# jiahuei/sparse-image-captioning

Hardware: AMD Instinct MI355X
Metric: captions/sec (higher is better)
Workload: dtype bf16; 1 GPU; configs[1]: ORT dense, 256 images x 5 captions, teacher-forcing XE fwd+bwd+clip+Adam; images_per_gpu=256, regions=36, captions_per_image=5, parallelism=single

## Files before the change

include/ortk.h:

```cpp
#ifndef ORTK_H
#define ORTK_H

#include <stddef.h>
#include <stdint.h>

#ifdef __cplusplus
extern "C" {
#endif

#define ORTK_VERSION 14
#define ORTK_EINVAL (-1)
#define ORTK_ENOSPC (-2)
#define ORTK_ENOSYS (-3)
#define ORTK_EEXCHANGE (-4)

typedef void* ortk_stream;

int ortk_version(void);
int ortk_device_ok(void);

struct ortk_sparse_plan;
typedef struct ortk_config {
    int32_t d_model, d_ff, n_layers, n_heads;
    int32_t vocab, feat, seq_len;
    int32_t pad_id, bos_id, eos_id, unk_id;
    int32_t box_trig;
    int32_t precision;
    float   drop_src, drop;
    int32_t share_enc[16], share_dec[16];
    int32_t share_att_enc, share_att_dec;
    int32_t no_box;
    const struct ortk_sparse_plan* sparse_fwd;
    const struct ortk_sparse_plan* sparse_bwd;
} ortk_config;

int64_t ortk_arena_numel(const ortk_config* cfg);
int64_t ortk_arena_numel_with_buffers(const ortk_config* cfg);
int32_t ortk_arena_entries(const ortk_config* cfg);
int ortk_arena_entry(const ortk_config* cfg, int32_t index, char* name_buf, int64_t* offset,
                     int64_t* numel, int32_t* ndim, int64_t* shape, int32_t* kind);

uint32_t ortk_dropout_site_seed(uint64_t seed, int32_t stack, int32_t layer, int32_t k);

// ... 97 lines not shown
typedef struct ortk_bchain_args {
    const void* w16t; const ortk_chain_unit* units_dev; int32_t n_units;
    void* packed; size_t packed_bytes;
    int64_t M;
    int32_t nin; const void* ain; int64_t ld_ain; const void* dz0;
    const float *xa, *sta, *ga, *dresa; float *dxa, *daa, *dba; void* dza; uint32_t seed_a; int32_t mask_a;
    int32_t NC; const void* hgate; void* gh; float gate_scale;
    const float *xb, *stb, *gb, *dresb; float *dxb, *dab, *dbb; void* dzb; uint32_t seed_b; int32_t mask_b;
    int32_t n2; void* out2;
    float drop_p, eps;
    const int32_t* drop_rows;
} ortk_bchain_args;
int ortk_row_bchain(const ortk_bchain_args* a, ortk_stream stream);

typedef struct ortk_tuning {
    int32_t gemm_t64;
    int32_t attn_impl;
    int32_t attn16_min_lq;
    int32_t side_stream;
    int32_t row_chain;
    int32_t chain_wide;
    int32_t spmm_alias;
    int32_t f32_split;
    int32_t wgrad_wgs;
    int32_t wgrad_group;
    int32_t wgrad_group_splitk;
    int32_t wgrad_group_wgs;
    int32_t wgrad_group_tail;
    int32_t feats_bf16;
    int32_t ln_fuse;
    int32_t samp_epilogue;
    int32_t gemm_epilogue;
    int32_t attn16_short;
} ortk_tuning;
void ortk_get_tuning(ortk_tuning* out);
int ortk_set_tuning(const ortk_tuning* t);

#define ORTK_DEC_UNFUSED 1
#define ORTK_DEC_STACK 2
#define ORTK_DEC_SPARSE_STREAM 4
#define ORTK_DEC_STACK_RB20 8
#define ORTK_DEC_STACK_SPLIT 16
#define ORTK_DEC_SPLIT_SMALL 32
#define ORTK_DEC_SPARSE_GATHER 64
#define ORTK_DEC_STACK_FP8 128
#define ORTK_MAX_BEAM 32
typedef struct ortk_decode_opts {
    int32_t beam_size;
    int32_t num_random_sample;
    float   temperature;
    int32_t decoding_constraint;
    int32_t length_penalty;
    double  length_alpha;
    uint64_t seed;
    const struct ortk_sparse_plan* sparse;
    int32_t exec_flags;
    int32_t with_greedy;
    int64_t sample_row_offset;
    int32_t train;
    uint64_t drop_seed;
    const void* memory;
    int32_t top_k;
    float   top_p;
    int32_t group_size;
    float   diversity_lambda;
} ortk_decode_opts;
// ... 195 lines not shown
```

sparse-image-captioning_amd/_lib.py:

```python
import ctypes as C
import os

import torch

_HERE = os.path.dirname(os.path.abspath(__file__))
LIB_PATH = os.path.join(_HERE, "libortk.so")


class OrtkUnavailable(RuntimeError):
    pass


class OrtkError(RuntimeError):
    pass


class Config(C.Structure):
    _fields_ = [("d_model", C.c_int32), ("d_ff", C.c_int32), ("n_layers", C.c_int32), ("n_heads", C.c_int32),
                ("vocab", C.c_int32), ("feat", C.c_int32), ("seq_len", C.c_int32),
                ("pad_id", C.c_int32), ("bos_id", C.c_int32), ("eos_id", C.c_int32), ("unk_id", C.c_int32),
                ("box_trig", C.c_int32), ("precision", C.c_int32), ("drop_src", C.c_float), ("drop", C.c_float),
                ("share_enc", C.c_int32 * 16), ("share_dec", C.c_int32 * 16),
                ("share_att_enc", C.c_int32), ("share_att_dec", C.c_int32), ("no_box", C.c_int32),
                ("sparse_fwd", C.c_void_p), ("sparse_bwd", C.c_void_p)]
# ... 50 lines not shown
                ("M", C.c_int64),
                ("nin", C.c_int32), ("ain", C.c_void_p), ("ld_ain", C.c_int64), ("dz0", C.c_void_p),
                ("xa", C.c_void_p), ("sta", C.c_void_p), ("ga", C.c_void_p), ("dresa", C.c_void_p), ("dxa", C.c_void_p), ("daa", C.c_void_p),
                ("dba", C.c_void_p), ("dza", C.c_void_p), ("seed_a", C.c_uint32), ("mask_a", C.c_int32),
                ("NC", C.c_int32), ("hgate", C.c_void_p), ("gh", C.c_void_p), ("gate_scale", C.c_float),
                ("xb", C.c_void_p), ("stb", C.c_void_p), ("gb", C.c_void_p), ("dresb", C.c_void_p), ("dxb", C.c_void_p), ("dab", C.c_void_p),
                ("dbb", C.c_void_p), ("dzb", C.c_void_p), ("seed_b", C.c_uint32), ("mask_b", C.c_int32),
                ("n2", C.c_int32), ("out2", C.c_void_p), ("drop_p", C.c_float), ("eps", C.c_float), ("drop_rows", C.c_void_p)]


class MaskedAdamArgs(C.Structure):
    _fields_ = [("w", C.c_void_p), ("g", C.c_void_p), ("mw", C.c_void_p), ("vw", C.c_void_p),
                ("ml", C.c_void_p), ("mm", C.c_void_p), ("mv", C.c_void_p),
                ("draws", C.c_void_p), ("active", C.c_void_p), ("extra_coef", C.c_void_p),
                ("n", C.c_int64), ("index0", C.c_int64), ("mode", C.c_int32), ("seed", C.c_uint32),
                ("lr_w", C.c_float), ("eps_w", C.c_float), ("lr_m", C.c_float), ("eps_m", C.c_float),
                ("beta1", C.c_float), ("beta2", C.c_float), ("clip", C.c_float), ("bc1", C.c_float), ("bc2", C.c_float)]


OPT_ADAM, OPT_SGD, OPT_SGDM, OPT_SGDMOM, OPT_RMSPROP, OPT_ADAGRAD = range(6)
OPT_KINDS = {"adam": OPT_ADAM, "sgd": OPT_SGD, "sgdm": OPT_SGDM, "sgdmom": OPT_SGDMOM, "rmsprop": OPT_RMSPROP, "adagrad": OPT_ADAGRAD}


class OptimArgs(C.Structure):
    _fields_ = [("p", C.c_void_p), ("g", C.c_void_p), ("s1", C.c_void_p), ("s2", C.c_void_p), ("n", C.c_int64),
                ("kind", C.c_int32), ("first_step", C.c_int32), ("zero_grad", C.c_int32),
                ("lr", C.c_float), ("weight_decay", C.c_float), ("alpha", C.c_float), ("beta", C.c_float), ("eps", C.c_float),
                ("clip", C.c_float), ("bc1", C.c_float), ("bc2", C.c_float)]


class Tuning(C.Structure):
    _fields_ = [("gemm_t64", C.c_int32), ("attn_impl", C.c_int32), ("attn16_min_lq", C.c_int32),
                ("side_stream", C.c_int32), ("row_chain", C.c_int32), ("chain_wide", C.c_int32), ("spmm_alias", C.c_int32), ("f32_split", C.c_int32), ("wgrad_wgs", C.c_int32),
                ("wgrad_group", C.c_int32), ("wgrad_group_splitk", C.c_int32), ("wgrad_group_wgs", C.c_int32), ("wgrad_group_tail", C.c_int32), ("feats_bf16", C.c_int32), ("ln_fuse", C.c_int32), ("samp_epilogue", C.c_int32), ("gemm_epilogue", C.c_int32), ("attn16_short", C.c_int32)]


MAX_BEAM = 32
DEC_UNFUSED, DEC_STACK, DEC_SPARSE_STREAM, DEC_STACK_RB20, DEC_STACK_SPLIT, DEC_SPLIT_SMALL, DEC_SPARSE_GATHER, DEC_STACK_FP8 = 1, 2, 4, 8, 16, 32, 64, 128


class DecodeOpts(C.Structure):
    _fields_ = [("beam_size", C.c_int32), ("num_random_sample", C.c_int32), ("temperature", C.c_float),
                ("decoding_constraint", C.c_int32), ("length_penalty", C.c_int32), ("length_alpha", C.c_double),
                ("seed", C.c_uint64), ("sparse", C.POINTER(EllPlanStruct)), ("exec_flags", C.c_int32), ("with_greedy", C.c_int32), ("sample_row_offset", C.c_int64),
                ("train", C.c_int32), ("drop_seed", C.c_uint64), ("memory", C.c_void_p), ("top_k", C.c_int32), ("top_p", C.c_float),
                ("group_size", C.c_int32), ("diversity_lambda", C.c_float)]


class GemmArgs(C.Structure):
    _fields_ = [("A", C.c_void_p), ("B", C.c_void_p), ("C", C.c_void_p),
                ("lda", C.c_int64), ("ldb", C.c_int64), ("ldc", C.c_int64),
                ("M", C.c_int32), ("N", C.c_int32), ("K", C.c_int32), ("transA", C.c_int32), ("transB", C.c_int32),
                ("bias", C.c_void_p), ("rowscale", C.c_void_p), ("resid", C.c_void_p), ("ldr", C.c_int64),
                ("gate", C.c_void_p), ("ldg", C.c_int64), ("gate_scale", C.c_float),
                ("relu", C.c_int32), ("drop_p", C.c_float), ("drop_seed", C.c_uint32),
                ("accumulate", C.c_int32), ("splitk", C.c_int32), ("precision", C.c_int32),
                ("a_dtype", C.c_int32), ("b_dtype", C.c_int32), ("c_dtype", C.c_int32), ("gate_dtype", C.c_int32),
                ("colsum", C.c_void_p), ("drop_row_stride", C.c_int32), ("drop_row_off", C.c_int32),
                ("ln_mode", C.c_int32), ("ln_y_dtype", C.c_int32),
                ("ln_a", C.c_void_p), ("ln_b", C.c_void_p), ("ln_y", C.c_void_p), ("ln_stats", C.c_void_p), ("ln_eps", C.c_float),
                ("ln_x", C.c_void_p), ("ln_dres", C.c_void_p), ("ln_da", C.c_void_p), ("ln_db", C.c_void_p),
                ("tile_stats", C.c_void_p), ("stat_ncols", C.c_int32), ("drop_rows", C.c_void_p),
                ("tile_samp", C.c_void_p), ("samp_seq", C.c_void_p), ("samp_seed", C.c_uint64), ("samp_row_offset", C.c_int64),
                ("samp_L", C.c_int32), ("samp_t", C.c_int32), ("samp_greedy_stride", C.c_int32), ("samp_sample", C.c_int32),
                ("samp_fast", C.c_int32), ("samp_no_store", C.c_int32), ("samp_inv_temperature", C.c_float)]


# ... 90 lines not shown
    "ortk_colsum": (_I32, [_P, _I32, _I64, _P, _I64, _I32, _P]),
    "ortk_gate_apply": (_I32, [_P, _P, _P, _I32, _I64, _F, _P]),
    "ortk_dropout_apply": (_I32, [_P, _P, _I32, _I64, _F, _U32, _P]),
    "ortk_dropout_apply_rows": (_I32, [_P, _P, _I32, _I64, _I32, _F, _U32, _P, _P]),
    "ortk_dropout_site_seed": (_U32, [_U64, _I32, _I32, _I32]),
    "ortk_cast_bf16": (_I32, [_P, _P, _I64, _P]),
    "ortk_fp8_rows": (_I32, [_P, _I64, _I64, _I64, _P, _I64, _P, _P, _I64, _P]),
    "ortk_fill": (_I32, [_P, _I64, _F, _P]),
    "ortk_sum_scratch_floats": (_I64, [_I64]),
    "ortk_sum": (_I32, [_P, _I64, _P, _P, _P]),
    "ortk_adam_clip": (_I32, [_P, _P, _P, _P, _I64, _F, _F, _F, _F, _F, _F, _F, _P]),
    "ortk_adam_clip_zero": (_I32, [_P, _P, _P, _P, _I64, _F, _F, _F, _F, _F, _F, _F, _P]),
    "ortk_optim_states": (_I32, [_I32]),
    "ortk_optim_step": (_I32, [C.POINTER(OptimArgs), _P]),
    "ortk_mask_apply": (_I32, [_P, _P, _P, _I64, _I32, _U32, _P]),
    "ortk_mask_bwd": (_I32, [_P, _P, _P, _P, _P, _I64, _I32, _U32, _P, _P]),
    "ortk_masked_adam_step": (_I32, [C.POINTER(MaskedAdamArgs), _P]),
    "ortk_mask_count": (_I32, [_P, _I64, _I32, _P, _P]),
    "ortk_mask_select_workspace_bytes": (_SZ, [_I32, _I32, _I32, _I32]),
    "ortk_mask_select": (_I32, [_P, _P, _P, _P, _P, _P, _P, _P, _P, _I32, _I32, _I32, _I32, _P, _SZ, _P]),
    "ortk_mask_apply_draws": (_I32, [_P, _P, _P, _P, _I64, _P]),
    "ortk_mask_bwd_draws": (_I32, [_P, _P, _P, _P, _P, _P, _I64, _P, _P]),
    "ortk_decode_step_workspace_bytes": (_SZ, [_CFG, _I32]),
    "ortk_project_memory": (_I32, [_CFG, _P, _P, _I64, _P, _SZ, _P, _P]),
    "ortk_decode_step": (_I32, [_CFG, _P, _P, _I32, _I32, _I32, _I32, _P, _P, _P, _P, _I32, _P, _SZ, _P, _I64, _P]),
    "ortk_axpy_cols": (_I32, [_P, _P, _I32, _I64, _I64, _I32, _P]),
    "ortk_linear_block": (_I32, [_CFG, _I32, C.POINTER(C.c_int64), C.POINTER(C.c_int32), C.POINTER(C.c_int32)]),
    "ortk_sparse_build": (_I32, [C.POINTER(EllPlanStruct), _P, _I32, _P]),
    "ortk_spmm": (_I32, [C.POINTER(EllPlanStruct), _I32, C.POINTER(SpmmArgs), _P]),
    "ortk_spmm_plan": (_I32, [C.POINTER(EllPlanStruct), _I32, C.POINTER(SpmmArgs), C.c_char_p, _I32]),
}

_lib = None
ABI_VERSION = 14


def lib():
    global _lib
    if _lib is None:
        if not os.path.exists(LIB_PATH):
            raise OrtkUnavailable(
                f"{LIB_PATH} is missing: build it with `python -c 'import __graft_entry__ as g; g.build()'` "
                "(or `make -C sparse-image-captioning_amd/csrc`).  There is no CPU / PyTorch fallback.")
        h = C.CDLL(LIB_PATH)
        h.ortk_version.restype = C.c_int32
        if h.ortk_version() != ABI_VERSION:
            raise OrtkUnavailable(
                f"{LIB_PATH} is ABI version {h.ortk_version()}, these bindings were written for version {ABI_VERSION} (include/ortk.h: "
                "ORTK_VERSION): a stale build.  Rebuild it with `make -C sparse-image-captioning_amd/csrc`.")
        for name, (res, args) in SIGNATURES.items():
            fn = getattr(h, name)
            fn.restype = res
            fn.argtypes = args
        _lib = h
    return _lib


def set_tuning(**kw):
    t = Tuning()
    lib().ortk_get_tuning(C.byref(t))
    old = {f: getattr(t, f) for f, _ in Tuning._fields_}
    for k, v in kw.items():
        assert k in old, k
        setattr(t, k, int(v))
    check(lib().ortk_set_tuning(C.byref(t)), "ortk_set_tuning")
    return old

# ... 50 lines not shown
```

sparse-image-captioning_amd/csrc/ortk_attn16.hip:

```cpp
#include <cstdlib>
#include "ortk_internal.h"

namespace {

constexpr int P16 = 72;

__device__ __forceinline__ void wsync() { __builtin_amdgcn_fence(__ATOMIC_ACQ_REL, "wavefront"); __builtin_amdgcn_wave_barrier(); }

template <int NJT> struct KeyGeo {
    static constexpr int KJ = NJT <= 2 ? 32 : NJT <= 4 ? 64 : NJT <= 6 ? 96 : 128;
    static constexpr int PJ = NJT <= 4 ? P16 : 136;
};

template <int PITCH = P16>
__device__ __forceinline__ bf16x8 frag_row(const __bf16* img, int row, int k0) {
    return *reinterpret_cast<const bf16x8*>(img + row * PITCH + k0);
}
template <int PITCH = P16>
__device__ __forceinline__ bf16x8 frag_tr(const __bf16* img, int k0, int x0, int lane) {
    const int lr = lane & 15, lq = lane >> 4;
    const __bf16* p = img + (k0 + 8 * lq + (lr >> 2)) * PITCH + x0 + 4 * (lane & 3);
    typedef bf16x4 __attribute__((address_space(3))) * lds4;
    const bf16x4 lo = __builtin_amdgcn_ds_read_tr16_b64_v4bf16((lds4)(p));
    const bf16x4 hi = __builtin_amdgcn_ds_read_tr16_b64_v4bf16((lds4)(p + 4 * PITCH));
// ... 237 lines not shown
        const int i = it * 16 + lr;
        iv[it] = i < Lqg;
        prow[it] = (((int64_t)g * a.H + h) * Lq + i) * Lk;
        drow[it] = prow[it];
        if (a.drop_p > 0.f && a.drop_rows && a.q_off && iv[it])
            drow[it] = (((int64_t)g * a.H + h) * Lq + ((int64_t)a.drop_rows[qrow0 + i] - (int64_t)g * Lq)) * Lk;
#pragma unroll
        for (int ks = 0; ks < NKS; ++ks) qf[it][ks] = (bf16x8){0, 0, 0, 0, 0, 0, 0, 0};
        if (iv[it]) {
            const __bf16* qp = aq + (qrow0 + i) * a.ldq + h * DK + 8 * lq;
#pragma unroll
            for (int ks = 0; ks < NKS; ++ks) qf[it][ks] = ld_frag(qp + 32 * ks);
        }
        ld_keys4<NJT>(bias4[it], a.bias, a.bias && iv[it], prow[it], Lk, lq);
    }
    stage32_st<DKT>(sV, vreg, lane);
    if (lane < 32) sMask[lane] = mk;
    for (int idx = lane; idx < 16 * (KJS / 4); idx += 64)
        *reinterpret_cast<bf16x4*>(sP + (idx / (KJS / 4)) * PJS + (idx % (KJS / 4)) * 4) = cvt4(make_float4(0.f, 0.f, 0.f, 0.f));
    wsync();
    const float inv_keep = a.drop_p > 0.f ? 1.f / (1.f - a.drop_p) : 1.f;
#pragma unroll
    for (int it = 0; it < 2; ++it) {
        if (it * 16 >= Lqg) break;
        fwd16_tile<NJT, DKT, PJS>(a, kf, qf[it], bias4[it], sMask, sV, sP, lane, it * 16 + lr, iv[it], prow[it], drow[it],
                                  qrow0 + it * 16 + lr, h, inv_keep);
        wsync();
    }
}
static int key_kj(int njt) { return njt <= 2 ? 32 : njt <= 4 ? 64 : njt <= 6 ? 96 : 128; }
static int key_pj(int njt) { return njt <= 4 ? P16 : 136; }
static size_t fwd16_lds(int njt, int nw, int dk) {
    return ((size_t)(16 * njt + key_kj(njt)) * (dk + 8) + (size_t)16 * nw * key_pj(njt)) * sizeof(__bf16) + 128 * sizeof(float);
}

template <int NJT, int DKT, int PJ, typename VF>
__device__ __forceinline__ void bwd16_tile1(const ortk_attn_args& a, const VF& vfr, const bf16x8 (&gf)[DKT / 32], const float4 (&praw)[NJT],
                                            const __bf16* sK, __bf16* sS, __bf16* sD, int lane, int i, bool iv,
                                            int64_t prow, int64_t drow, int64_t qrow, int h, float inv_keep) {
    constexpr int DK = DKT, PD = DKT + 8, KJ = KeyGeo<NJT>::KJ;
    const float qscale = DKT == 64 ? 0.125f : 0.17677669529663687f;
    const int lq = lane >> 4, Lk = a.Lk;
    const bool vec_p = (Lk & 3) == 0;
    f32x4 dp[NJT], pp[NJT];
    float dot = 0.f;
#pragma unroll
    for (int jt = 0; jt < NJT; ++jt) {
        dp[jt] = (f32x4){0.f, 0.f, 0.f, 0.f};
#pragma unroll
        for (int ks = 0; ks < DK / 32; ++ks) dp[jt] = mma(vfr(jt, ks), gf[ks], dp[jt]);
        const int j0 = 16 * jt + 4 * lq;
        const float pv[4] = {praw[jt].x, praw[jt].y, praw[jt].z, praw[jt].w};
        float pd[4];
        bool kp[4] = {true, true, true, true};
        if (a.drop_p > 0.f) ortk_keep4(a.drop_seed, (uint64_t)(drow + j0), a.drop_p, kp);
#pragma unroll
        for (int r = 0; r < 4; ++r) {
            const bool valid = iv && j0 + r < Lk;
            const bool keep = valid && kp[r];
            const float d = keep ? dp[jt][r] * inv_keep : 0.f;
            pd[r] = keep ? pv[r] * inv_keep : 0.f;
            pp[jt][r] = valid ? pv[r] : 0.f; dp[jt][r] = d; dot += pp[jt][r] * d;
        }
        *reinterpret_cast<bf16x4*>(sD + i * PJ + j0) = cvt4(make_float4(pd[0], pd[1], pd[2], pd[3]));
    }
    dot += __shfl_xor(dot, 16, 64); dot += __shfl_xor(dot, 32, 64);
// ... 135 lines not shown
        }
        ld_keys4<NJT>(praw[it], a.p, iv[it], prow[it], Lk, lq);
    }
    bf16x8 kreg[DKT / 16], qreg[DKT / 16], greg[DKT / 16];
    stage32_ld<DKT>(kreg, ak + krow0 * a.ldk + h * DK, a.ldk, Lkg, lane);
    stage32_ld<DKT>(qreg, aq + qrow0 * a.ldq + h * DK, a.ldq, Lqg, lane);
    stage32_ld<DKT>(greg, ag + qrow0 * a.lddo + h * DK, a.lddo, Lqg, lane);
    for (int idx = lane; idx < 2 * LQP * PJS / 8; idx += 64)
        *reinterpret_cast<bf16x8*>(sS + idx * 8) = (bf16x8){0, 0, 0, 0, 0, 0, 0, 0};
    stage32_st<DKT>(sX, kreg, lane);
    wsync();
    const float inv_keep = a.drop_p > 0.f ? 1.f / (1.f - a.drop_p) : 1.f;
#pragma unroll
    for (int it = 0; it < 2; ++it) {
        if (it * 16 >= Lqg) break;
        bwd16_tile1<NJT, DKT, PJS>(a, vf, gf[it], praw[it], sX, sS, sD, lane, it * 16 + lr, iv[it], prow[it], drow[it],
                                   qrow0 + it * 16 + lr, h, inv_keep);
    }
    constexpr int NDT = DK / 16;
#pragma unroll
    for (int which = 0; which < 2; ++which) {
        wsync();
        stage32_st<DKT>(sX, which == 0 ? qreg : greg, lane);
        wsync();
        for (int jt = 0; jt < NJT && 16 * jt < Lkg; ++jt)
            for (int dt = 0; dt < NDT; ++dt)
                bwd16_tile2<NJT, DKT, PJS>(a, (which * NJT + jt) * NDT + dt, sS, sD, sX, sX, LQP, lane, Lkg, krow0, h);
    }
}
static size_t bwd16_lds(int njt, int Lqp, int dk) {
    return ((size_t)(key_kj(njt) + 16 * njt + 2 * Lqp) * (dk + 8) + (size_t)2 * Lqp * key_pj(njt)) * sizeof(__bf16);
}

bool al16(const void* p) { return (reinterpret_cast<uintptr_t>(p) & 15) == 0; }

}

namespace ortk {

bool attn16_shape_ok(int Lq, int Lk, int dk) { return (dk == 64 || dk == 32) && Lk >= 1 && Lk <= 128 && Lq >= 1 && Lq <= 128; }

bool attn16_ok(const ortk_attn_args* a, bool bwd) {
    const int min_lq = ortk::tuning().attn16_min_lq;
    if (a->precision != 1 || !attn16_shape_ok(a->Lq, a->Lk, a->dk) || (a->qkv_dtype == 0 && a->Lq < min_lq && a->Lk <= 48)) return false;
    if (a->kv_index || a->kv_group_stride > 0 || a->kv_dtype != 0 || a->k_new || a->v_new) return false;
    if (a->q_off && (a->qkv_dtype != 1 || a->q_off_stride < 1)) return false;
    if ((a->ldq | a->ldk | a->ldv) % (a->qkv_dtype ? 8 : 4) || !al16(a->q) || !al16(a->k) || !al16(a->v)) return false;
    if (!bwd) {
        const int64_t eo = a->o_dtype == ORTK_BF16 ? 2 : 4;
        if (a->ldo % 4 || (reinterpret_cast<uintptr_t>(a->o) % (4 * eo)) || (a->p && !al16(a->p)) || (a->bias && !al16(a->bias))) return false;
    } else {
        const int64_t eg = a->dqkv_dtype == ORTK_BF16 ? 2 : 4;
        if (!a->p || !a->d_o || !a->dq || !a->d_k || !a->dv) return false;
        if ((a->lddo % (a->qkv_dtype ? 8 : 4)) || (a->lddq | a->lddk | a->lddv) % 4 || !al16(a->d_o) || !al16(a->p) || (a->dscore && !al16(a->dscore))) return false;
        if ((reinterpret_cast<uintptr_t>(a->dq) | reinterpret_cast<uintptr_t>(a->d_k) | reinterpret_cast<uintptr_t>(a->dv)) % (4 * eg)) return false;
    }
    return true;
}

typedef void (*fwd16_fn)(ortk_attn_args);
typedef void (*bwd16_fn)(ortk_attn_args, int);
template <typename TQ, int DKT> static fwd16_fn pick_fwd(int njt) {
    switch (njt) {
        case 1: return attn16_fwd_kernel<1, TQ, DKT>; case 2: return attn16_fwd_kernel<2, TQ, DKT>; case 3: return attn16_fwd_kernel<3, TQ, DKT>;
        case 4: return attn16_fwd_kernel<4, TQ, DKT>; case 5: return attn16_fwd_kernel<5, TQ, DKT>; case 6: return attn16_fwd_kernel<6, TQ, DKT>;
        case 7: return attn16_fwd_kernel<7, TQ, DKT>; default: return attn16_fwd_kernel<8, TQ, DKT>;
    }
}
template <typename TQ, int DKT> static bwd16_fn pick_bwd(int njt) {
    switch (njt) {
        case 1: return attn16_bwd_kernel<1, TQ, DKT>; case 2: return attn16_bwd_kernel<2, TQ, DKT>; case 3: return attn16_bwd_kernel<3, TQ, DKT>;
        case 4: return attn16_bwd_kernel<4, TQ, DKT>; case 5: return attn16_bwd_kernel<5, TQ, DKT>; case 6: return attn16_bwd_kernel<6, TQ, DKT>;
        case 7: return attn16_bwd_kernel<7, TQ, DKT>; default: return attn16_bwd_kernel<8, TQ, DKT>;
    }
}

static int short_waves(const ortk_attn_args* a) {
    const int sw = ortk::tuning().attn16_short;
    if (!sw || a->qkv_dtype != 1 || a->Lq > 32 || a->Lk > 32) return 0;
    return sw == 8 ? 8 : 4;
}
template <typename FN> static int launch_short(FN fn, size_t wave_bytes, int W, const ortk_attn_args* a, hipStream_t s) {
    const size_t lds = wave_bytes * W;
    const int64_t pairs = (int64_t)a->nkv * a->H;
    if (lds > 64 * 1024) ortk::lds_attr(reinterpret_cast<const void*>(fn), 160 * 1024);
    hipLaunchKernelGGL(fn, dim3((unsigned)((pairs + W - 1) / W)), dim3(64 * W), lds, s, *a);
    ORTK_CHECK_LAUNCH();
    return 0;
}

int attn16_fwd(const ortk_attn_args* a, hipStream_t s) {
    if (const int W = short_waves(a)) {
        const bool two = a->Lk > 16;
        const fwd16_fn fn = a->dk == 64 ? (two ? attn16s_fwd_kernel<2, 64> : attn16s_fwd_kernel<1, 64>) : (two ? attn16s_fwd_kernel<2, 32> : attn16s_fwd_kernel<1, 32>);
        return launch_short(fn, (a->dk == 64 ? fwd16s_wave_elems<64>() : fwd16s_wave_elems<32>()) * sizeof(__bf16), W, a, s);
    }
    const int njt = (a->Lk + 15) / 16, nw = (a->Lq + 15) / 16;
    const fwd16_fn fn = a->dk == 64 ? (a->qkv_dtype ? pick_fwd<__bf16, 64>(njt) : pick_fwd<float, 64>(njt))
                                    : (a->qkv_dtype ? pick_fwd<__bf16, 32>(njt) : pick_fwd<float, 32>(njt));
    const size_t lds = fwd16_lds(njt, nw, a->dk);
    if (lds > 64 * 1024) ortk::lds_attr(reinterpret_cast<const void*>(fn), 160 * 1024);
    hipLaunchKernelGGL(fn, dim3((unsigned)(a->nkv * a->H)), dim3(64 * nw), lds, s, *a);
    ORTK_CHECK_LAUNCH();
    return 0;
}

int attn16_bwd(const ortk_attn_args* a, hipStream_t s) {
    if (const int W = short_waves(a)) {
        const bool two = a->Lk > 16;
        const fwd16_fn fn = a->dk == 64 ? (two ? attn16s_bwd_kernel<2, 64> : attn16s_bwd_kernel<1, 64>) : (two ? attn16s_bwd_kernel<2, 32> : attn16s_bwd_kernel<1, 32>);
        return launch_short(fn, (a->dk == 64 ? bwd16s_wave_elems<64>() : bwd16s_wave_elems<32>()) * sizeof(__bf16), W, a, s);
    }
    const int njt = (a->Lk + 15) / 16, nw = (a->Lq + 15) / 16, Lqp = (int)ortk_align(a->Lq, 32);
    const bwd16_fn fn = a->dk == 64 ? (a->qkv_dtype ? pick_bwd<__bf16, 64>(njt) : pick_bwd<float, 64>(njt))
                                    : (a->qkv_dtype ? pick_bwd<__bf16, 32>(njt) : pick_bwd<float, 32>(njt));
    const size_t lds = bwd16_lds(njt, Lqp, a->dk);
    if (lds > 160 * 1024) return ORTK_EINVAL;
    if (lds > 64 * 1024) ortk::lds_attr(reinterpret_cast<const void*>(fn), 160 * 1024);
    hipLaunchKernelGGL(fn, dim3((unsigned)(a->nkv * a->H)), dim3(64 * nw), lds, s, *a, Lqp);
    ORTK_CHECK_LAUNCH();
    return 0;
}

}
```

sparse-image-captioning_amd/csrc/ortk_runtime.hip:

```cpp
#include <mutex>
#include <vector>
#include "ortk_internal.h"

namespace ortk {
static ortk_tuning tuning_defaults() {
    ortk_tuning t{};
    t.gemm_t64 = 640;
    t.attn_impl = 0;
    t.attn16_min_lq = 33;
    t.side_stream = 1;
    t.row_chain = 1;
    t.chain_wide = 1;
    t.spmm_alias = 1;
    t.f32_split = 1;
    t.wgrad_wgs = 384;
    t.wgrad_group = 3;
    t.wgrad_group_splitk = 0;
    t.wgrad_group_wgs = 80;
    t.wgrad_group_tail = 1;
    t.feats_bf16 = 1;
    t.ln_fuse = 0;
    t.samp_epilogue = 1;
    t.gemm_epilogue = 0;
    t.attn16_short = 1;
    return t;
}
static ortk_tuning g_tuning = tuning_defaults();
const ortk_tuning& tuning() { return g_tuning; }
}

extern "C" void ortk_get_tuning(ortk_tuning* out) { if (out) *out = ortk::g_tuning; }
extern "C" int ortk_set_tuning(const ortk_tuning* t) {
    if (!t) return ORTK_EINVAL;
    auto in = [](int32_t v, int32_t lo, int32_t hi) { return v >= lo && v <= hi; };
    if (!in(t->attn_impl, 0, 4) || t->attn16_min_lq < 1 || !in(t->f32_split, 0, 7) || t->wgrad_wgs < 1 ||
        !in(t->wgrad_group, 0, 15) || !in(t->wgrad_group_splitk, 0, 8) || t->wgrad_group_wgs < 1 || !in(t->wgrad_group_tail, 0, 1) ||
        !in(t->feats_bf16, 0, 1) || !in(t->ln_fuse, 0, 15) || (t->ln_fuse & 2)  ||
        !in(t->samp_epilogue, 0, 1) || !in(t->gemm_epilogue, 0, 3) ||
        !(in(t->attn16_short, 0, 1) || t->attn16_short == 4 || t->attn16_short == 8)) return ORTK_EINVAL;
    ortk::g_tuning = *t;
    return 0;
}

namespace ortk {
int lds_attr(const void* fn, size_t bytes) {
    struct Key { int dev; const void* fn; size_t bytes; };
    static std::mutex mu;
    static std::vector<Key>* seen = new std::vector<Key>();
    int dev = 0;
    if (hipGetDevice(&dev) != hipSuccess) return ORTK_EINVAL;
    std::lock_guard<std::mutex> lk(mu);
    for (const Key& k : *seen) if (k.dev == dev && k.fn == fn && k.bytes >= bytes) return 0;
    if (hipFuncSetAttribute(fn, hipFuncAttributeMaxDynamicSharedMemorySize, (int)bytes) != hipSuccess) return ORTK_EINVAL;
    seen->push_back(Key{dev, fn, bytes});
    return 0;
}
}

namespace {
struct ProfRec { hipEvent_t a, b; int key; double flops, bytes; int slot; double per_count; double units; };
constexpr int PROF_SLOTS = 1 << 16;
unsigned long long* g_prof_slots = nullptr;
int g_prof_slot_next = 0;
bool g_prof_on = false;
bool g_prof_serial = false;
std::mutex g_prof_mu;
std::vector<ProfRec>* g_prof = nullptr;
}

namespace ortk {
bool ortk_prof_active() { return g_prof_on; }
bool ortk_prof_serial() { return g_prof_serial; }
// ... 73 lines not shown
```

Baseline: 133,700 captions/sec.

## Add block-per-head attn16 fwd/bwd kernels with three-wave workgroups

```diff
diff --git a/include/ortk.h b/include/ortk.h
--- a/include/ortk.h
+++ b/include/ortk.h
@@ -8,7 +8,7 @@
 extern "C" {
 #endif
 
-#define ORTK_VERSION 14
+#define ORTK_VERSION 15
 #define ORTK_EINVAL (-1)
 #define ORTK_ENOSPC (-2)
 #define ORTK_ENOSYS (-3)
@@ -172,6 +172,7 @@
     int32_t samp_epilogue;
     int32_t gemm_epilogue;
     int32_t attn16_short;
+    int32_t attn16_block;
 } ortk_tuning;
 void ortk_get_tuning(ortk_tuning* out);
 int ortk_set_tuning(const ortk_tuning* t);
diff --git a/scratch/attn16_block_bench.py b/scratch/attn16_block_bench.py
--- /dev/null
+++ b/scratch/attn16_block_bench.py
@@ -0,0 +1,95 @@
+import ctypes as C, hashlib, os, socket, sys
+import torch
+ROOT = os.path.dirname(os.path.dirname(os.path.abspath(__file__)))
+sys.path.insert(0, ROOT)
+import sparse_image_captioning_amd as P
+L = P._lib
+L.require_gpu()
+print("box", socket.gethostname(), " lib md5", hashlib.md5(open(L.LIB_PATH, "rb").read()).hexdigest(), flush=True)
+H, dk, S, T, spi = 8, 64, 36, 17, 5
+d = H * dk
+HAS = "attn16_block" in L.set_tuning()
+SETTINGS = (0, 1) if HAS else (0,)
+
+
+def setting(v):
+    if HAS: L.set_tuning(attn16_block=v)
+
+
+def build(kind, nimg):
+    g = torch.Generator().manual_seed(3)
+    Lq = S if kind == "enc" else spi * T
+    if kind == "crossv":
+        lengths = torch.randint(9, T + 1, (nimg * spi,), generator=torch.Generator().manual_seed(11)).tolist()
+    else:
+        lengths = None
+    off = [0]
+    for n in lengths or []: off.append(off[-1] + n)
+    Mq = off[-1] if lengths else nimg * Lq
+    Mk = nimg * S
+    a = L.AttnArgs()
+    a.precision, a.qkv_dtype, a.o_dtype, a.dqkv_dtype = 1, 1, 1, 1
+    hold = []
+    if kind == "enc":
+        qkv = torch.randn(Mq, 3 * d, generator=g).bfloat16().cuda(); dqkv = torch.empty(Mq, 3 * d, device="cuda", dtype=torch.bfloat16)
+        a.q, a.k, a.v = qkv.data_ptr(), qkv.data_ptr() + 2 * d, qkv.data_ptr() + 4 * d
+        a.ldq = a.ldk = a.ldv = 3 * d
+        a.dq, a.d_k, a.dv = dqkv.data_ptr(), dqkv.data_ptr() + 2 * d, dqkv.data_ptr() + 4 * d
+        a.lddq = a.lddk = a.lddv = 3 * d
+        bias = torch.randn(nimg, H, S, S, generator=g).cuda(); ds = torch.empty(nimg, H, S, S, device="cuda")
+        a.bias, a.dscore = bias.data_ptr(), ds.data_ptr()
+        outs = [dqkv, ds]; hold += [qkv, bias]
+    else:
+        q = torch.randn(Mq, d, generator=g).bfloat16().cuda(); kv = torch.randn(Mk, 2 * d, generator=g).bfloat16().cuda()
+        dq = torch.empty(Mq, d, device="cuda", dtype=torch.bfloat16); dkv = torch.empty(Mk, 2 * d, device="cuda", dtype=torch.bfloat16)
+        a.q, a.k, a.v = q.data_ptr(), kv.data_ptr(), kv.data_ptr() + 2 * d
+        a.ldq, a.ldk, a.ldv = d, 2 * d, 2 * d
+        a.dq, a.d_k, a.dv = dq.data_ptr(), dkv.data_ptr(), dkv.data_ptr() + 2 * d
+        a.lddq, a.lddk, a.lddv = d, 2 * d, 2 * d
+        outs = [dq, dkv]; hold += [q, kv]
+        if lengths:
+            qo = torch.tensor(off, dtype=torch.int32).cuda()
+            rp = torch.tensor([c * T + t for c, n in enumerate(lengths) for t in range(n)], dtype=torch.int32).cuda()
+            a.q_off, a.q_off_stride, a.drop_rows = qo.data_ptr(), spi, rp.data_ptr()
+            hold += [qo, rp]
+    do = torch.randn(Mq, d, generator=g).bfloat16().cuda(); o = torch.empty(Mq, d, device="cuda", dtype=torch.bfloat16)
+    p = torch.zeros(nimg, H, Lq, S, device="cuda"); km = torch.ones(Mk, device="cuda")
+    a.o, a.p, a.kmask, a.ldo, a.d_o, a.lddo = o.data_ptr(), p.data_ptr(), km.data_ptr(), d, do.data_ptr(), d
+    a.nkv, a.H, a.Lq, a.Lk, a.dk, a.drop_p, a.drop_seed = nimg, H, Lq, S, dk, 0.1, 5
+    return a, [o, p] + outs, hold + [do, km]
+
+
+def md5s(ts):
+    torch.cuda.synchronize()
+    return [hashlib.md5(t.cpu().contiguous().view(torch.int16 if t.element_size() == 2 else torch.int32).numpy().tobytes()).hexdigest() for t in ts]
+
+
+def timed(fn, a, n=50):
+    for _ in range(3): L.check(fn(C.byref(a), L.stream_ptr()), "attention")
+    torch.cuda.synchronize()
+    e0, e1 = torch.cuda.Event(enable_timing=True), torch.cuda.Event(enable_timing=True)
+    e0.record()
+    for _ in range(n): fn(C.byref(a), L.stream_ptr())
+    e1.record(); torch.cuda.synchronize()
+    return e0.elapsed_time(e1) * 1000.0 / n
+
+
+def case(kind, nimg, rounds=3):
+    a, outs, hold = build(kind, nimg)
+    fns = (("fwd", L.lib().ortk_attention_fwd), ("bwd", L.lib().ortk_attention_bwd))
+    res, sums = {}, {}
+    for rep in range(rounds):
+        for sw in SETTINGS:
+            setting(sw)
+            for fname, fn in fns: res.setdefault((sw, fname), []).append(timed(fn, a))
+            sums[sw] = md5s(outs)
+    setting(1)
+    for sw in SETTINGS:
+        print(f"{kind:6s} {nimg:4d} images  attn16_block={sw}: fwd us {' '.join(f'{x:6.1f}' for x in res[(sw, 'fwd')])}   bwd us {' '.join(f'{x:6.1f}' for x in res[(sw, 'bwd')])}"
+              f"   outputs {'== attn16_block=0' if sums[sw] == sums[0] else 'DIFFER'}", flush=True)
+
+
+if len(sys.argv) > 1 and sys.argv[1] == "sweep":
+    for n in (96, 192, 200, 256, 384): case("enc", n)
+else:
+    for kind in ("enc", "cross", "crossv"): case(kind, 256)
diff --git a/sparse-image-captioning_amd/_lib.py b/sparse-image-captioning_amd/_lib.py
--- a/sparse-image-captioning_amd/_lib.py
+++ b/sparse-image-captioning_amd/_lib.py
@@ -106,7 +106,7 @@
 class Tuning(C.Structure):
     _fields_ = [("gemm_t64", C.c_int32), ("attn_impl", C.c_int32), ("attn16_min_lq", C.c_int32),
                 ("side_stream", C.c_int32), ("row_chain", C.c_int32), ("chain_wide", C.c_int32), ("spmm_alias", C.c_int32), ("f32_split", C.c_int32), ("wgrad_wgs", C.c_int32),
-                ("wgrad_group", C.c_int32), ("wgrad_group_splitk", C.c_int32), ("wgrad_group_wgs", C.c_int32), ("wgrad_group_tail", C.c_int32), ("feats_bf16", C.c_int32), ("ln_fuse", C.c_int32), ("samp_epilogue", C.c_int32), ("gemm_epilogue", C.c_int32), ("attn16_short", C.c_int32)]
+                ("wgrad_group", C.c_int32), ("wgrad_group_splitk", C.c_int32), ("wgrad_group_wgs", C.c_int32), ("wgrad_group_tail", C.c_int32), ("feats_bf16", C.c_int32), ("ln_fuse", C.c_int32), ("samp_epilogue", C.c_int32), ("gemm_epilogue", C.c_int32), ("attn16_short", C.c_int32), ("attn16_block", C.c_int32)]
 
 
 MAX_BEAM = 32
@@ -263,7 +263,7 @@
 }
 
 _lib = None
-ABI_VERSION = 14
+ABI_VERSION = 15
 
 
 def lib():
diff --git a/sparse-image-captioning_amd/csrc/ortk_attn16.hip b/sparse-image-captioning_amd/csrc/ortk_attn16.hip
--- a/sparse-image-captioning_amd/csrc/ortk_attn16.hip
+++ b/sparse-image-captioning_amd/csrc/ortk_attn16.hip
@@ -293,6 +293,113 @@
 static int key_pj(int njt) { return njt <= 4 ? P16 : 136; }
 static size_t fwd16_lds(int njt, int nw, int dk) {
     return ((size_t)(16 * njt + key_kj(njt)) * (dk + 8) + (size_t)16 * nw * key_pj(njt)) * sizeof(__bf16) + 128 * sizeof(float);
+}
+
+constexpr int NWB = 3, NTB = 64 * NWB;
+template <int DKT, int ROWS> struct StageB { static constexpr int N = (ROWS * (DKT / 8) + NTB - 1) / NTB; };
+template <int DKT, int ROWS, int N = StageB<DKT, ROWS>::N>
+__device__ __forceinline__ void stageb_ld(bf16x8 (&v)[N], const __bf16* src, int64_t ld, int rows, int tid) {
+    constexpr int CPR = DKT / 8;
+#pragma unroll
+    for (int n = 0; n < N; ++n) {
+        const int idx = tid + NTB * n, r = idx / CPR, c = (idx % CPR) * 8;
+        v[n] = (bf16x8){0, 0, 0, 0, 0, 0, 0, 0};
+        if (r < rows) v[n] = *reinterpret_cast<const bf16x8*>(src + ((unsigned)r * (unsigned)ld + (unsigned)c));
+    }
+}
+template <int NJT, int NKS>
+__device__ __forceinline__ void ld_row_fragsb(RegRowFrags<NJT, NKS>& out, const __bf16* src, int64_t ld, int rows, int lane) {
+    const int lr = lane & 15, lq = lane >> 4;
+#pragma unroll
+    for (int jt = 0; jt < NJT; ++jt)
+#pragma unroll
+        for (int ks = 0; ks < NKS; ++ks) {
+            out.f[jt][ks] = (bf16x8){0, 0, 0, 0, 0, 0, 0, 0};
+            if (16 * jt + lr < rows) out.f[jt][ks] = ld_frag(src + ((unsigned)(16 * jt + lr) * (unsigned)ld + (unsigned)(32 * ks + 8 * lq)));
+        }
+}
+template <int DKT, int ROWS, int N = StageB<DKT, ROWS>::N>
+__device__ __forceinline__ void stageb_st(__bf16* img, const bf16x8 (&v)[N], int rows_st, int tid) {
+    constexpr int CPR = DKT / 8;
+#pragma unroll
+    for (int n = 0; n < N; ++n) {
+        const int idx = tid + NTB * n, r = idx / CPR, c = (idx % CPR) * 8;
+        if (r < rows_st) *reinterpret_cast<bf16x8*>(img + r * (DKT + 8) + c) = v[n];
+    }
+}
+template <int NJT, int DKT, int TPW>
+__global__ __launch_bounds__(NTB) __attribute__((amdgpu_waves_per_eu(NJT * DKT > 192 ? 4 : 6))) void attn16b_fwd_kernel(ortk_attn_args a) {
+    static_assert(NJT <= 4 && TPW <= 2, "at most 64 keys and 96 query rows");
+    constexpr int DK = DKT, PD = DKT + 8, NKS = DKT / 32, KJ = KeyGeo<NJT>::KJ, PJ = KeyGeo<NJT>::PJ;
+    const __bf16* aq = reinterpret_cast<const __bf16*>(a.q); const __bf16* ak = reinterpret_cast<const __bf16*>(a.k); const __bf16* av = reinterpret_cast<const __bf16*>(a.v);
+    extern __shared__ __attribute__((aligned(16))) __bf16 sm16[];
+    const int tid = threadIdx.x, lane = tid & 63, wave = __builtin_amdgcn_readfirstlane(tid >> 6);
+    const int g = blockIdx.x / a.H, h = blockIdx.x - g * a.H;
+    const int Lk = a.Lk, Lq = a.Lq;
+    constexpr int KP = 16 * NJT * PD > NWB * 16 * PJ ? 16 * NJT * PD : NWB * 16 * PJ;
+    __bf16* sV = sm16;
+    __bf16* sK = sV + KJ * PD;
+    __bf16* sP = sK + wave * 16 * PJ;
+    float* sMask = reinterpret_cast<float*>(sK + KP);
+    const int lr = lane & 15, lq = lane >> 4;
+    int64_t qrow0 = (int64_t)g * Lq;
+    int Lqg = Lq;
+    if (a.q_off) {
+        const int o0 = a.q_off[(int64_t)g * a.q_off_stride], o1 = a.q_off[(int64_t)(g + 1) * a.q_off_stride];
+        qrow0 = o0; Lqg = min(Lq, o1 - o0);
+    }
+    const int64_t krow0 = (a.q_off && a.kv_ragged) ? qrow0 : (int64_t)g * Lk;
+    const int Lkg = (a.q_off && a.kv_ragged) ? min(Lk, Lqg) : Lk;
+    bf16x8 vreg[StageB<DKT, KJ>::N];
+    stageb_ld<DKT, KJ>(vreg, av + krow0 * a.ldv + h * DK, a.ldv, Lkg, tid);
+    float mk = -1.f;
+    if (tid < Lkg) mk = a.kmask ? a.kmask[krow0 + tid] : 1.f;
+    bf16x8 kreg[StageB<DKT, 16 * NJT>::N];
+    stageb_ld<DKT, 16 * NJT>(kreg, ak + krow0 * a.ldk + h * DK, a.ldk, Lkg, tid);
+    bf16x8 qf[TPW][NKS];
+    float4 bias4[TPW][NJT];
+    int64_t prow[TPW], drow[TPW];
+    bool iv[TPW];
+#pragma unroll
+    for (int t = 0; t < TPW; ++t) {
+        const int i = (wave + NWB * t) * 16 + lr;
+        iv[t] = i < Lqg;
+        prow[t] = (((int64_t)g * a.H + h) * Lq + i) * Lk;
+        drow[t] = prow[t];
+        if (a.drop_p > 0.f && a.drop_rows && a.q_off && iv[t])
+            drow[t] = (((int64_t)g * a.H + h) * Lq + ((int64_t)a.drop_rows[qrow0 + i] - (int64_t)g * Lq)) * Lk;
+#pragma unroll
+        for (int ks = 0; ks < NKS; ++ks) qf[t][ks] = (bf16x8){0, 0, 0, 0, 0, 0, 0, 0};
+        if (iv[t]) {
+            const __bf16* qp = aq + qrow0 * a.ldq + h * DK + ((unsigned)i * (unsigned)a.ldq + (unsigned)(8 * lq));
+#pragma unroll
+            for (int ks = 0; ks < NKS; ++ks) qf[t][ks] = ld_frag(qp + 32 * ks);
+        }
+        ld_keys4<NJT>(bias4[t], a.bias, TPW == 1 && a.bias && iv[t], prow[t], Lk, lq);
+    }
+    stageb_st<DKT, KJ>(sV, vreg, KJ, tid);
+    stageb_st<DKT, 16 * NJT>(sK, kreg, 16 * NJT, tid);
+    if (tid < 64) sMask[tid] = mk;
+    __syncthreads();
+    RegRowFrags<NJT, NKS> kf;
+#pragma unroll
+    for (int jt = 0; jt < NJT; ++jt)
+#pragma unroll
+        for (int ks = 0; ks < NKS; ++ks) kf.f[jt][ks] = frag_row<PD>(sK, 16 * jt + lr, 32 * ks + 8 * lq);
+    __syncthreads();
+    for (int idx = lane; idx < 16 * (KJ / 4); idx += 64)
+        *reinterpret_cast<bf16x4*>(sP + (idx / (KJ / 4)) * PJ + (idx % (KJ / 4)) * 4) = cvt4(make_float4(0.f, 0.f, 0.f, 0.f));
+    const float inv_keep = a.drop_p > 0.f ? 1.f / (1.f - a.drop_p) : 1.f;
+#pragma unroll
+    for (int t = 0; t < TPW; ++t) {
+        const int i0 = (wave + NWB * t) * 16;
+        if (i0 >= Lqg) break;
+        if (t) wsync();
+        fwd16_tile<NJT, DKT, PJ>(a, kf, qf[t], bias4[t], sMask, sV, sP, lane, i0 + lr, iv[t], prow[t], drow[t], qrow0 + i0 + lr, h, inv_keep);
+    }
+}
+static size_t fwd16b_lds(int njt, int dk) {
+    return ((size_t)key_kj(njt) * (dk + 8) + std::max((size_t)16 * njt * (dk + 8), (size_t)16 * NWB * key_pj(njt))) * sizeof(__bf16) + 64 * sizeof(float);
 }
 
 template <int NJT, int DKT, int PJ, typename VF>
@@ -494,6 +601,81 @@
     return ((size_t)(key_kj(njt) + 16 * njt + 2 * Lqp) * (dk + 8) + (size_t)2 * Lqp * key_pj(njt)) * sizeof(__bf16);
 }
 
+template <int NJT, int DKT, int TPW>
+__global__ __launch_bounds__(NTB) void attn16b_bwd_kernel(ortk_attn_args a, int Lqp) {
+    static_assert(NJT <= 4 && TPW <= 2, "at most 64 keys and 96 query rows");
+    constexpr int DK = DKT, PD = DKT + 8, NKS = DKT / 32, KJ = KeyGeo<NJT>::KJ, PJ = KeyGeo<NJT>::PJ;
+    constexpr int LQM = TPW == 1 ? 64 : 96;
+    const __bf16* aq = reinterpret_cast<const __bf16*>(a.q); const __bf16* ak = reinterpret_cast<const __bf16*>(a.k); const __bf16* av = reinterpret_cast<const __bf16*>(a.v);
+    const __bf16* ag = reinterpret_cast<const __bf16*>(a.d_o);
+    extern __shared__ __attribute__((aligned(16))) __bf16 sm16[];
+    const int tid = threadIdx.x, lane = tid & 63, wave = __builtin_amdgcn_readfirstlane(tid >> 6);
+    const int g = blockIdx.x / a.H, h = blockIdx.x - g * a.H;
+    const int Lk = a.Lk, Lq = a.Lq;
+    __bf16* sX = sm16;
+    __bf16* sS = sX + max(KJ, Lqp) * PD;
+    __bf16* sD = sS + Lqp * PJ;
+    const int lr = lane & 15, lq = lane >> 4;
+    int64_t qrow0 = (int64_t)g * Lq;
+    int Lqg = Lq;
+    if (a.q_off) {
+        const int o0 = a.q_off[(int64_t)g * a.q_off_stride], o1 = a.q_off[(int64_t)(g + 1) * a.q_off_stride];
+        qrow0 = o0; Lqg = min(Lq, o1 - o0);
+    }
+    const int64_t krow0 = (a.q_off && a.kv_ragged) ? qrow0 : (int64_t)g * Lk;
+    const int Lkg = (a.q_off && a.kv_ragged) ? min(Lk, Lqg) : Lk;
+    RegRowFrags<NJT, NKS> vf;
+    ld_row_fragsb<NJT, NKS>(vf, av + krow0 * a.ldv + h * DK, a.ldv, Lkg, lane);
+    bf16x8 gf[TPW][NKS];
+    float4 praw[TPW][NJT];
+    int64_t prow[TPW], drow[TPW];
+    bool iv[TPW];
+#pragma unroll
+    for (int t = 0; t < TPW; ++t) {
+        const int i = (wave + NWB * t) * 16 + lr;
+        iv[t] = i < Lqg;
+        prow[t] = (((int64_t)g * a.H + h) * Lq + i) * Lk;
+        drow[t] = prow[t];
+        if (a.drop_p > 0.f && a.drop_rows && a.q_off && iv[t])
+            drow[t] = (((int64_t)g * a.H + h) * Lq + ((int64_t)a.drop_rows[qrow0 + i] - (int64_t)g * Lq)) * Lk;
+#pragma unroll
+        for (int ks = 0; ks < NKS; ++ks) gf[t][ks] = (bf16x8){0, 0, 0, 0, 0, 0, 0, 0};
+        if (iv[t]) {
+            const __bf16* gp = ag + qrow0 * a.lddo + h * DK + ((unsigned)i * (unsigned)a.lddo + (unsigned)(8 * lq));
+#pragma unroll
+            for (int ks = 0; ks < NKS; ++ks) gf[t][ks] = ld_frag(gp + 32 * ks);
+        }
+        ld_keys4<NJT>(praw[t], a.p, iv[t], prow[t], Lk, lq);
+    }
+    bf16x8 kreg[StageB<DKT, KJ>::N], qreg[StageB<DKT, LQM>::N], greg[StageB<DKT, LQM>::N];
+    stageb_ld<DKT, KJ>(kreg, ak + krow0 * a.ldk + h * DK, a.ldk, Lkg, tid);
+    stageb_ld<DKT, LQM>(qreg, aq + qrow0 * a.ldq + h * DK, a.ldq, Lqg, tid);
+    stageb_ld<DKT, LQM>(greg, ag + qrow0 * a.lddo + h * DK, a.lddo, Lqg, tid);
+    for (int idx = tid; idx < 2 * Lqp * PJ / 8; idx += NTB)
+        *reinterpret_cast<bf16x8*>(sS + idx * 8) = (bf16x8){0, 0, 0, 0, 0, 0, 0, 0};
+    stageb_st<DKT, KJ>(sX, kreg, KJ, tid);
+    __syncthreads();
+    const float inv_keep = a.drop_p > 0.f ? 1.f / (1.f - a.drop_p) : 1.f;
+#pragma unroll
+    for (int t = 0; t < TPW; ++t) {
+        const int i0 = (wave + NWB * t) * 16;
+        if (i0 >= Lqg) break;
+        bwd16_tile1<NJT, DKT, PJ>(a, vf, gf[t], praw[t], sX, sS, sD, lane, i0 + lr, iv[t], prow[t], drow[t], qrow0 + i0 + lr, h, inv_keep);
+    }
+    constexpr int NT2 = NJT * (DK / 16);
+    const int Lq2 = min(Lqp, (Lqg + 31) & ~31);
+#pragma unroll
+    for (int which = 0; which < 2; ++which) {
+        __syncthreads();
+        stageb_st<DKT, LQM>(sX, which == 0 ? qreg : greg, Lqp, tid);
+        __syncthreads();
+        for (int t = wave; t < NT2; t += NWB) bwd16_tile2<NJT, DKT, PJ>(a, which * NT2 + t, sS, sD, sX, sX, Lq2, lane, Lkg, krow0, h);
+    }
+}
+static size_t bwd16b_lds(int njt, int Lqp, int dk) {
+    return ((size_t)std::max(key_kj(njt), Lqp) * (dk + 8) + (size_t)2 * Lqp * key_pj(njt)) * sizeof(__bf16);
+}
+
 bool al16(const void* p) { return (reinterpret_cast<uintptr_t>(p) & 15) == 0; }
 
 }
@@ -542,6 +724,21 @@
     if (!sw || a->qkv_dtype != 1 || a->Lq > 32 || a->Lk > 32) return 0;
     return sw == 8 ? 8 : 4;
 }
+static bool block_b(const ortk_attn_args* a) {
+    return ortk::tuning().attn16_block && a->qkv_dtype == 1 && a->Lk <= 64 && a->Lq <= 16 * NWB * 2 && (a->Lq <= 16 * NWB || !a->bias);
+}
+template <int DKT, int TPW> static fwd16_fn pick_fwd_b(int njt) {
+    switch (njt) {
+        case 1: return attn16b_fwd_kernel<1, DKT, TPW>; case 2: return attn16b_fwd_kernel<2, DKT, TPW>;
+        case 3: return attn16b_fwd_kernel<3, DKT, TPW>; default: return attn16b_fwd_kernel<4, DKT, TPW>;
+    }
+}
+template <int DKT, int TPW> static bwd16_fn pick_bwd_b(int njt) {
+    switch (njt) {
+        case 1: return attn16b_bwd_kernel<1, DKT, TPW>; case 2: return attn16b_bwd_kernel<2, DKT, TPW>;
+        case 3: return attn16b_bwd_kernel<3, DKT, TPW>; default: return attn16b_bwd_kernel<4, DKT, TPW>;
+    }
+}
 template <typename FN> static int launch_short(FN fn, size_t wave_bytes, int W, const ortk_attn_args* a, hipStream_t s) {
     const size_t lds = wave_bytes * W;
     const int64_t pairs = (int64_t)a->nkv * a->H;
@@ -558,6 +755,12 @@
         return launch_short(fn, (a->dk == 64 ? fwd16s_wave_elems<64>() : fwd16s_wave_elems<32>()) * sizeof(__bf16), W, a, s);
     }
     const int njt = (a->Lk + 15) / 16, nw = (a->Lq + 15) / 16;
+    if (block_b(a)) {
+        const fwd16_fn fn = a->dk == 64 ? (nw <= NWB ? pick_fwd_b<64, 1>(njt) : pick_fwd_b<64, 2>(njt)) : (nw <= NWB ? pick_fwd_b<32, 1>(njt) : pick_fwd_b<32, 2>(njt));
+        hipLaunchKernelGGL(fn, dim3((unsigned)(a->nkv * a->H)), dim3(NTB), fwd16b_lds(njt, a->dk), s, *a);
+        ORTK_CHECK_LAUNCH();
+        return 0;
+    }
     const fwd16_fn fn = a->dk == 64 ? (a->qkv_dtype ? pick_fwd<__bf16, 64>(njt) : pick_fwd<float, 64>(njt))
                                     : (a->qkv_dtype ? pick_fwd<__bf16, 32>(njt) : pick_fwd<float, 32>(njt));
     const size_t lds = fwd16_lds(njt, nw, a->dk);
@@ -574,6 +777,12 @@
         return launch_short(fn, (a->dk == 64 ? bwd16s_wave_elems<64>() : bwd16s_wave_elems<32>()) * sizeof(__bf16), W, a, s);
     }
     const int njt = (a->Lk + 15) / 16, nw = (a->Lq + 15) / 16, Lqp = (int)ortk_align(a->Lq, 32);
+    if (block_b(a)) {
+        const bwd16_fn fn = a->dk == 64 ? (nw <= NWB ? pick_bwd_b<64, 1>(njt) : pick_bwd_b<64, 2>(njt)) : (nw <= NWB ? pick_bwd_b<32, 1>(njt) : pick_bwd_b<32, 2>(njt));
+        hipLaunchKernelGGL(fn, dim3((unsigned)(a->nkv * a->H)), dim3(NTB), bwd16b_lds(njt, Lqp, a->dk), s, *a, Lqp);
+        ORTK_CHECK_LAUNCH();
+        return 0;
+    }
     const bwd16_fn fn = a->dk == 64 ? (a->qkv_dtype ? pick_bwd<__bf16, 64>(njt) : pick_bwd<float, 64>(njt))
                                     : (a->qkv_dtype ? pick_bwd<__bf16, 32>(njt) : pick_bwd<float, 32>(njt));
     const size_t lds = bwd16_lds(njt, Lqp, a->dk);
diff --git a/sparse-image-captioning_amd/csrc/ortk_runtime.hip b/sparse-image-captioning_amd/csrc/ortk_runtime.hip
--- a/sparse-image-captioning_amd/csrc/ortk_runtime.hip
+++ b/sparse-image-captioning_amd/csrc/ortk_runtime.hip
@@ -23,6 +23,7 @@
     t.samp_epilogue = 1;
     t.gemm_epilogue = 0;
     t.attn16_short = 1;
+    t.attn16_block = 1;
     return t;
 }
 static ortk_tuning g_tuning = tuning_defaults();
@@ -37,7 +38,7 @@
         !in(t->wgrad_group, 0, 15) || !in(t->wgrad_group_splitk, 0, 8) || t->wgrad_group_wgs < 1 || !in(t->wgrad_group_tail, 0, 1) ||
         !in(t->feats_bf16, 0, 1) || !in(t->ln_fuse, 0, 15) || (t->ln_fuse & 2)  ||
         !in(t->samp_epilogue, 0, 1) || !in(t->gemm_epilogue, 0, 3) ||
-        !(in(t->attn16_short, 0, 1) || t->attn16_short == 4 || t->attn16_short == 8)) return ORTK_EINVAL;
+        !(in(t->attn16_short, 0, 1) || t->attn16_short == 4 || t->attn16_short == 8) || !in(t->attn16_block, 0, 1)) return ORTK_EINVAL;
     ortk::g_tuning = *t;
     return 0;
 }
```

Measured after the change: 135,700 captions/sec (median of 6 runs). +1.5%, better.
